# rrrickyz/Parallel-and-Distributed-Deep-Learning

Hardware: AMD Instinct MI355X
Metric: images/sec ResNet-50/ImageNet at 1/2/4/8 MI355X + scaling efficiency (higher is better)
Workload: dtype bf16; 1 GPU; model=ResNet-50 Keras-v1 (25,636,712 params, random init), global_batch=2560, per_gpu_batch=2560, image_size=224, parallelism=dp1, replicas=1, optimizer=adam, bn=frozen (training=False), hip_graph=False, grad_dtype=fp32, device=MI355X

## Files before the change

### csrc/bindings.cpp

```cpp
#include <torch/extension.h>

#include <atomic>
#include <ATen/hip/HIPContext.h>
#include <ATen/hip/impl/HIPGuardImplMasqueradingAsCUDA.h>
#include <c10/util/Optional.h>

#include "kernels/kernels.h"

using torch::Tensor;
using OptT = c10::optional<Tensor>;
namespace py = pybind11;

#define PCHECK(cond, msg) TORCH_CHECK(cond, "pddl: ", msg)

namespace {

std::atomic<bool> g_launched{false};
std::atomic<bool> g_knob_tuning{false};
hipStream_t cur_stream() {
  if (!g_launched.load(std::memory_order_relaxed)) g_launched.store(true, std::memory_order_relaxed);
  return at::hip::getCurrentHIPStream().stream();
}

void ok(const char* err, const char* what) { TORCH_CHECK(err == nullptr, "pddl ", what, ": ", err ? err : ""); }
// ... 802 lines not shown
  m.def("conv3x3c64_wgrad", &conv3x3c64_wgrad, REL, py::arg("x"), py::arg("g"), py::arg("dw"));
  m.def("c3c1", &c3c1, REL, py::arg("a"), py::arg("w3"), py::arg("scale3"), py::arg("shift3"),
        py::arg("res"), py::arg("out"), py::arg("bits3"), py::arg("w1"), py::arg("scale1"), py::arg("shift1"),
        py::arg("y1"), py::arg("bits1"));
  m.def("conv3x3c64_partial_rows", [](int64_t M) { return pddl::conv3x3c64_partial_rows((int)M); });
  m.def("gap_fwd", &gap_fwd, REL);
  m.def("gap_bwd", &gap_bwd, REL);
  m.def("colsum", &colsum, REL);
  m.def("softmax_xent", &softmax_xent, REL);
  m.def("eval_metrics", &eval_metrics, REL);
  m.def("colsum_reduce", &colsum_reduce, REL);
  m.def("allow_knob_changes", [](bool on) { g_knob_tuning.store(on); }, py::arg("on") = true);
  m.def("knobs_frozen", []() { return g_launched.load() && !g_knob_tuning.load(); });
  m.def("set_variant", [](const std::string& which, int v) {
    TORCH_CHECK(!g_launched.load() || g_knob_tuning.load(), "kernel knob ", which,
                ": knobs are read-only once a kernel has launched (set them before the first launch, "
                "e.g. PDDL_KNOBS, or call allow_knob_changes(True) in tuning code)");
    if (which == "igemm") pddl::g_igemm_variant = v;
    else if (which == "igemm_deep") pddl::g_igemm_deep = v;
    else if (which == "igemm_pf") pddl::g_igemm_pf = v;
    else if (which == "igemm8") pddl::g_igemm8 = v;
    else if (which == "igemm8_min_tiles") pddl::g_igemm8_min_tiles = v;
    else if (which == "wgrad8") pddl::g_wgrad8 = v;
    else if (which == "igemm_ns1_kt") pddl::g_igemm_ns1_kt = v;
    else if (which == "igemm8_min_n") pddl::g_igemm8_min_n = v;
    else if (which == "wgrad1") pddl::g_wgrad1 = v;
    else if (which == "igemm_n64") pddl::g_igemm_n64 = v;
    else if (which == "igemm_splitk") pddl::g_igemm_splitk = v;
    else if (which == "igemm_sk_fill") { TORCH_CHECK(v >= 1 && v <= 8, "igemm_sk_fill: 1-8"); pddl::g_igemm_sk_fill = v; }
    else if (which == "igemm_sk_cap") { TORCH_CHECK(v >= 2 && v <= 16, "igemm_sk_cap: 2-16"); pddl::g_igemm_sk_cap = v; }
    else if (which == "igemm_sk_elig") { TORCH_CHECK(v >= 1 && v <= 8, "igemm_sk_elig: 1-8"); pddl::g_igemm_sk_elig = v; }
    else if (which == "igemm_pk_all") pddl::g_igemm_pk_all = v;
    else if (which == "igemm_pk_dual") pddl::g_igemm_pk_dual = v;
    else if (which == "igemm_pk") { TORCH_CHECK(v == 0 || (v >= 2 && v <= 4), "igemm_pk: 0 or ring depth 2-4"); pddl::g_igemm_pk = v; }
    else if (which == "wgrad8_min_rows") { TORCH_CHECK(v >= 64, "wgrad8_min_rows"); pddl::g_wgrad8_min_rows = v; }
    else if (which == "stem") pddl::g_stem_variant = v;
    else if (which == "conv_f32") pddl::g_conv_f32_variant = v;
    else if (which == "conv_f32_splitk") pddl::g_conv_f32_splitk = v;
    else if (which == "conv_f32_sk_elig") { TORCH_CHECK(v >= 1 && v <= 8, "conv_f32_sk_elig: 1-8"); pddl::g_conv_f32_sk_elig = v; }
    else if (which == "wgrad_f32_wpc64") { TORCH_CHECK(v >= 1 && v <= 32, "wgrad_f32_wpc64"); pddl::g_wgrad_f32_wpc[0] = v; }
    else if (which == "wgrad_f32_wpc128") { TORCH_CHECK(v >= 1 && v <= 32, "wgrad_f32_wpc128"); pddl::g_wgrad_f32_wpc[1] = v; }
    else if (which == "c64_grid") pddl::g_c64_grid = v;
    else if (which == "c64w_grid") pddl::g_c64w_grid = v;
    else if (which == "bn_red_blocks") pddl::g_bn_red_blocks = v;
    else if (which == "bn_apply_blocks") pddl::g_bn_apply_blocks = v;
    else if (which == "pool_blocks") pddl::g_pool_blocks = v;
    else if (which == "colred_chunks") { TORCH_CHECK(v >= 1 && v <= 65535, "colred_chunks"); pddl::g_colred_chunks = v; }
    else TORCH_CHECK(false, "unknown kernel knob ", which);
  });
  m.def("wgrad_last_tiling", []() { return pddl::g_wgrad_last_tiling; });
  m.def("stream_capture_deps", [](int64_t stream) {
    hipStreamCaptureStatus st = hipStreamCaptureStatusNone;
    unsigned long long id = 0;
    hipGraph_t g = nullptr;
    const hipGraphNode_t* deps = nullptr;
    size_t n = 0;
    const hipError_t e = hipStreamGetCaptureInfo_v2(reinterpret_cast<hipStream_t>(stream), &st, &id, &g, &deps, &n);
    return std::make_tuple((int)e, (int)st, (int64_t)n);
  });
  m.def("igemm_partial_rows", [](int M, int Nn, int K, bool bnz) { return pddl::igemm_partial_rows(M, Nn, K, bnz); },
        py::arg("M"), py::arg("Nn"), py::arg("K"), py::arg("bnz") = false);
  m.def("igemm_splitk_floats", [](int M, int Nn, int K) { return (int64_t)pddl::igemm_splitk_floats(M, Nn, K); });
  m.def("splitk_use", &splitk_use, py::arg("workspace"));
  m.def("splitk_default_floats", &splitk_default_floats, py::arg("device"));
  m.def("igemm_plan", [](int M, int Nn, int K) {
    int cfg = 0, split = 0, ks = 1;
    pddl::igemm_plan_query(M, Nn, K, &cfg, &split, &ks);
    return std::make_tuple(cfg, split, ks);
  });
  m.def("maxpool_bwd_partial_rows", &pddl::maxpool_bwd_partial_rows);
  m.attr("COLRED_LAYER_BYTES") = (int)sizeof(pddl::ColRedLayer);
  m.def("prep", &prep, REL, py::arg("params"), py::arg("table"), py::arg("nlayers"), py::arg("max_elems"),
        py::arg("wbf"), py::arg("scale"), py::arg("shift"), py::arg("eps"), py::arg("parts") = 3);
  m.def("prep_fuse", &prep_fuse, REL);
  m.def("wgrad_finalize", &wgrad_finalize, REL, py::arg("params"), py::arg("grads"), py::arg("table"),
        py::arg("nlayers"), py::arg("scale"), py::arg("dgamma_raw"), py::arg("max_cout") = 2048);
  m.def("bn_grad", &bn_grad, REL);
  m.def("synth", &synth, REL);
  m.def("opt_hparams", &opt_hparams, REL);
  m.def("adam", &adam, REL);
  m.def("sgd", &sgd, REL);
  m.def("scale_", &scale_, REL);
  m.def("cast_bf16", &cast_bf16, REL);
// ... 10 lines not shown
```

### csrc/kernels/igemm.hip

```cpp
#include "common.h"
#include "kernels.h"

namespace pddl {

enum { AM_DIRECT = 0, AM_HALO = 1, AM_DUAL = 2 };

#ifndef IGEMM_MIN_BLOCKS
#define IGEMM_MIN_BLOCKS 2
#endif

__device__ __forceinline__ int sw_chunk(int lane, int i) { return (lane & 7) ^ ((4 * (i & 1) + (lane >> 4)) & 7); }
__device__ __forceinline__ int sw_read(int lane, int kh) { return (((kh * 4) + (lane >> 4)) ^ ((lane >> 1) & 7)) * 16; }

__device__ __forceinline__ uint32_t halo_taps(const IgemmParams& p, int hi, int wi) {
  if (p.R == 3 && p.S == 3) {
    const uint32_t cols = ((unsigned)wi < (unsigned)p.W ? 1u : 0u) | ((unsigned)(wi + 1) < (unsigned)p.W ? 2u : 0u) |
                          ((unsigned)(wi + 2) < (unsigned)p.W ? 4u : 0u);
    return ((unsigned)hi < (unsigned)p.H ? cols : 0u) | ((unsigned)(hi + 1) < (unsigned)p.H ? cols << 3 : 0u) |
           ((unsigned)(hi + 2) < (unsigned)p.H ? cols << 6 : 0u);
  }
  uint32_t rows = 0, cols = 0, mk = 0;
  for (int r = 0; r < p.R; ++r) rows |= (uint32_t)((unsigned)(hi + r) < (unsigned)p.H) << r;
  for (int s = 0; s < p.S; ++s) cols |= (uint32_t)((unsigned)(wi + s) < (unsigned)p.W) << s;
  for (int r = 0; r < p.R; ++r) mk |= ((rows >> r) & 1u) ? cols << (r * p.S) : 0u;
// ... 356 lines not shown
      for (int i = 0; i < TM; ++i)
#pragma unroll
        for (int j = 0; j < TN; ++j)
          acc[i][j] = __builtin_amdgcn_mfma_f32_16x16x32_bf16(af[i], bfr[j], acc[i][j], 0, 0, 0);
    }
    if (NSTAGE == 1 && t + 1 < KT) {
      __syncthreads();
      load_tile(0);
    }
    asm volatile("s_waitcnt vmcnt(0)" ::: "memory");
    __syncthreads();
  }

  if constexpr (SK) {
    float4* dst = reinterpret_cast<float4*>(p.slab) + ((long)(wg * ks + slice) * NW + wave) * (TM * TN) * 64 + lane;
#pragma unroll
    for (int i = 0; i < TM; ++i)
#pragma unroll
      for (int j = 0; j < TN; ++j)
        dst[(i * TN + j) * 64] = make_float4(acc[i][j][0], acc[i][j][1], acc[i][j][2], acc[i][j][3]);
    return;
  }

  float* stage = reinterpret_cast<float*>(smem) + wave * (32 * (WTN + 4));
  igemm_epilogue<TM, TN, PF, BNZ>(p, acc, m0 + wm * WTM, n0 + wn * WTN, p.prow_begin + tm * (BM / WTM) + wm, stage,
                                  lane);
}


typedef unsigned int v4u_t __attribute__((ext_vector_type(4)));
__device__ __forceinline__ int cdiv_signed(int a, int b) { return a >= 0 ? (a + b - 1) / b : -((-a) / b); }
__device__ __forceinline__ int pk_sw(int row) { return (row & 3) | ((row & 4) << 1); }

template <int KT, int NB, bool OPS, bool FWD, bool DUAL = false>
__global__ void __launch_bounds__(256, NB == 2 ? 2 : 1) igemm_pk_kernel(IgemmParams p) {
  constexpr int BM = 128, BN = 128, NW = 4, TM = 4, TN = 4, WAVES_N = 2;
  constexpr int A_BYTES = BM * 128, STAGE = A_BYTES + BN * 128;
  constexpr int BITS_BYTES = BM * 16;
  constexpr int AI = BM / (8 * NW), BI = BN / (8 * NW), PPS = AI + BI;
  constexpr int SPT = KT + (OPS ? 1 : 0);
  static_assert(NB >= 2 && NB * (STAGE + (OPS ? BITS_BYTES : 0)) <= 160 * 1024, "ring must fit the LDS");
  __shared__ __attribute__((aligned(16))) char smem[NB * STAGE + (OPS ? NB * BITS_BYTES : 1)];
  char* bits_lds = smem + NB * STAGE;
  const int tid = threadIdx.x, lane = tid & 63;
  const int wave = __builtin_amdgcn_readfirstlane(tid >> 6);
  const int wm = wave / WAVES_N, wn = wave % WAVES_N;
  const int mt = (p.M - p.m_begin + BM - 1) / BM, nt = (p.Nn + BN - 1) / BN;
  const int T = mt * nt, G = gridDim.x;
  const int bq = xcd_remap(blockIdx.x, G);
  if (bq >= T) return;
  const int t_begin = bq, t_end = T;
  const long HW = (long)p.H * p.W, pix_end = p.N * HW;
  const long HW2 = DUAL ? (long)p.H2 * p.W2 : 0;
  const int KT1 = DUAL ? p.K1 / 64 : KT;
  const int HoWo = p.Ho * p.Wo;
  const __amdgpu_buffer_rsrc_t rb = make_rsrc(p.b, p.Nn * p.ldb * 2);

  constexpr bool is_fwd = FWD;
  const uint16_t* opnd = is_fwd ? p.res : p.add;
  const int ld_op = is_fwd ? p.ld_res : p.ld_add;
  const bool res_on = OPS && opnd != nullptr;
  const bool bits_in = OPS && !is_fwd && p.bits_mask != nullptr;
  const bool bits_out = is_fwd && p.bits_out != nullptr;
  const bool csum_on = !is_fwd && p.colsum != nullptr;
  const int op_n = (res_on ? 8 : 0) + (bits_in ? 2 : 0) + (is_fwd ? 1 : 0);
  const int e_n = 2 * TM * (bits_out ? 2 : 1) + (csum_on ? 2 : 0);

  int ld_t = t_begin, ld_j = 0;
  uint32_t a_o[AI], a_o2[DUAL ? AI : 1], b_o[BI];
  __amdgpu_buffer_rsrc_t ra, ra2;
  auto set_tile = [&](int t) {
    const int m0 = p.m_begin + (t / nt) * BM, n0 = (t % nt) * BN;
    const int n_first = fdiv(m0, p.mg_howo);
    ra = make_rsrc_at(p.a1, n_first * HW * p.C1, pix_end * p.C1);
    if (DUAL) ra2 = make_rsrc_at(p.a2, n_first * HW2 * p.C2, p.N * HW2 * p.C2);
#pragma unroll
    for (int i = 0; i < AI; ++i) {
      const int m = m0 + (wave * AI + i) * 8 + (lane >> 3);
      a_o[i] = OOB_OFF;
      if (DUAL) a_o2[i] = OOB_OFF;
      if (m < p.M) {
        const int n = fdiv(m, p.mg_howo), rem = m - n * HoWo;
        const int ho = fdiv(rem, p.mg_wo), wo = rem - ho * p.Wo;
        const int pix = ((n - n_first) * p.H + ho * p.stride) * p.W + wo * p.stride;
        a_o[i] = (uint32_t)((pix * p.C1 + sw_chunk(lane, i) * 8) * 2);
        if (DUAL) {
          const int pix2 = ((n - n_first) * p.H2 + ho * p.stride2) * p.W2 + wo * p.stride2;
          a_o2[i] = (uint32_t)((pix2 * p.C2 + sw_chunk(lane, i) * 8) * 2);
        }
      }
    }
#pragma unroll
    for (int i = 0; i < BI; ++i) {
      const int n = n0 + (wave * BI + i) * 8 + (lane >> 3);
      b_o[i] = (n < p.Nn) ? (uint32_t)((n * p.ldb + sw_chunk(lane, i) * 8) * 2) : OOB_OFF;
    }
  };
  set_tile(t_begin);
  auto issue = [&](int buf) {
    const bool live = ld_t < t_end;
    char* base = smem + buf * STAGE;
    if (!OPS || ld_j < KT) {
      const int kofs = ld_j * 128;
      if (DUAL && ld_j >= KT1) {
#pragma unroll
        for (int i = 0; i < AI; ++i)
          buf_lds16(ra2, LDS_PTR(base + (wave * AI + i) * 1024), live ? a_o2[i] : OOB_OFF, kofs - KT1 * 128);
      } else {
#pragma unroll
        for (int i = 0; i < AI; ++i) buf_lds16(ra, LDS_PTR(base + (wave * AI + i) * 1024), live ? a_o[i] : OOB_OFF, kofs);
      }
#pragma unroll
      for (int i = 0; i < BI; ++i)
        buf_lds16(rb, LDS_PTR(base + A_BYTES + (wave * BI + i) * 1024), live ? b_o[i] : OOB_OFF, kofs);
    } else {
      const int lt = live ? ld_t : t_begin;
      const int m0 = p.m_begin + (lt / nt) * BM, n0 = (lt % nt) * BN;
      if (res_on) {
        const __amdgpu_buffer_rsrc_t ro = make_rsrc_at(opnd, (long)m0 * ld_op, (long)p.M * ld_op);
#pragma unroll
        for (int i = 0; i < 8; ++i) {
          const int row = wave * 32 + i * 4 + (lane >> 4);
          const int ch = (lane & 15) ^ pk_sw(row);
          const int col = n0 + ch * 8;
          const bool ok = live && m0 + row < p.M && col < p.Nn;
          buf_lds16(ro, LDS_PTR(base + (wave * 32 + i * 4) * 256), ok ? (uint32_t)((row * ld_op + col) * 2) : OOB_OFF, 0);
        }
      }
      if (is_fwd) {
        const float* src = wave < 2 ? p.scale : p.shift;
        const __amdgpu_buffer_rsrc_t rs = make_rsrc(src, p.Nn * 4);
        const int col = n0 + (wave & 1) * 64 + lane;
        __builtin_amdgcn_raw_ptr_buffer_load_lds(rs, LDS_PTR(bits_lds + buf * BITS_BYTES + wave * 256), 4,
                                                 live && col < p.Nn ? (uint32_t)(col * 4) : OOB_OFF, 0, 0, 0);
      }
      if (bits_in) {
        const int ldb8 = p.ld_bits_mask;
        const __amdgpu_buffer_rsrc_t rbm =
            __builtin_amdgcn_make_buffer_rsrc(const_cast<uint8_t*>(p.bits_mask) + (long)m0 * ldb8, (short)0,
                                              (int)lmin(((long)p.M - m0) * ldb8, 0x7fffffffL), 0x00020000);
#pragma unroll
        for (int q = 0; q < 2; ++q) {
          const int row = wave * 32 + q * 16 + (lane >> 2);
          const int byte = (n0 >> 3) + (lane & 3) * 4;
          const bool ok = live && m0 + row < p.M && byte * 8 < p.Nn;
          __builtin_amdgcn_raw_ptr_buffer_load_lds(rbm, LDS_PTR(bits_lds + buf * BITS_BYTES + (wave * 32 + q * 16) * 16), 4,
                                                   ok ? (uint32_t)(row * ldb8 + byte) : OOB_OFF, 0, 0, 0);
        }
      }
    }
    if (++ld_j == SPT) {
      ld_j = 0;
      ld_t += G;
      if (ld_t < t_end) set_tile(ld_t);
    }
  };
  auto wait_barrier = [&](int younger) {
    switch ((younger > 63 ? 63 : younger) >> 2) {
#define PK_W(n, c) case n: asm volatile("s_waitcnt vmcnt(" #c ") lgkmcnt(0)\n\ts_barrier" ::: "memory"); break;
      PK_W(1, 4) PK_W(2, 8) PK_W(3, 12) PK_W(4, 16) PK_W(5, 20) PK_W(6, 24) PK_W(7, 28) PK_W(8, 32) PK_W(9, 36)
      PK_W(10, 40) PK_W(11, 44) PK_W(12, 48) PK_W(13, 52) PK_W(14, 56) PK_W(15, 60)
#undef PK_W
      default: asm volatile("s_waitcnt vmcnt(0) lgkmcnt(0)\n\ts_barrier" ::: "memory"); break;
    }
  };

#pragma unroll
  for (int j = 0; j < NB - 1; ++j) issue(j);
  int cur = 0;
  const int a_off = (wm * 64 + (lane & 15)) * 128;
  const int b_off = (wn * 64 + (lane & 15)) * 128;
  const int g = lane >> 4, r = lane & 15, r8 = r & 7;
  const int lc = wn * 64 + 32 * (r >> 3) + 16 * (g & 1) + 8 * (g >> 1);
  for (int t = t_begin, u = 0; t < t_end; t += G, ++u) {
    const int m0 = p.m_begin + (t / nt) * BM, n0 = (t % nt) * BN;
    v4f acc[TM][TN];
#pragma unroll
    for (int i = 0; i < TM; ++i)
#pragma unroll
      for (int j = 0; j < TN; ++j) acc[i][j] = v4f{0.f, 0.f, 0.f, 0.f};
    int op_slot = 0;
#pragma unroll
    for (int j = 0; j < SPT; ++j) {
      int y = 0;
#pragma unroll
      for (int x = 1; x <= NB - 2; ++x) y += (OPS && (j + x) % SPT == KT) ? op_n : PPS;
      int ce = 1 - cdiv_signed(j - NB + 2, SPT);
      ce = ce < 0 ? 0 : (ce > u ? u : ce);
      wait_barrier(y + ce * e_n);
      issue(cur == 0 ? NB - 1 : cur - 1);
      if (!OPS || j < KT) {
        const char* As = smem + cur * STAGE;
        const char* Bs = As + A_BYTES;
#pragma unroll
        for (int kh = 0; kh < 2; ++kh) {
          const int pos = sw_read(lane, kh);
          v8bf af[TM], bfr[TN];
#pragma unroll
          for (int i = 0; i < TM; ++i) af[i] = *reinterpret_cast<const v8bf*>(As + a_off + i * 16 * 128 + pos);
#pragma unroll
          for (int jn = 0; jn < TN; ++jn) bfr[jn] = *reinterpret_cast<const v8bf*>(Bs + b_off + jn * 16 * 128 + pos);
#pragma unroll
          for (int i = 0; i < TM; ++i)
#pragma unroll
            for (int jn = 0; jn < TN; ++jn)
              acc[i][jn] = __builtin_amdgcn_mfma_f32_16x16x32_bf16(bfr[jn], af[i], acc[i][jn], 0, 0, 0);
        }
      } else {
        op_slot = cur;
      }
      cur = cur + 1 == NB ? 0 : cur + 1;
    }

#pragma unroll
    for (int i = 0; i < TM; ++i) {
#pragma unroll
      for (int q = 0; q < 2; ++q)
#pragma unroll
        for (int jj = 0; jj < 4; ++jj) {
          const auto sw = __builtin_amdgcn_permlane16_swap(__float_as_uint(acc[i][2 * q][jj]),
                                                           __float_as_uint(acc[i][2 * q + 1][jj]), false, false);
          acc[i][2 * q][jj] = __uint_as_float(sw[0]);
          acc[i][2 * q + 1][jj] = __uint_as_float(sw[1]);
        }
#pragma unroll
      for (int j = 0; j < 2; ++j)
#pragma unroll
        for (int jj = 0; jj < 4; ++jj) {
          const int c0 = __float_as_int(acc[i][j][jj]), c1 = __float_as_int(acc[i][2 + j][jj]);
          acc[i][j][jj] = __int_as_float(__builtin_amdgcn_update_dpp(c0, c1, 0x128, 0xf, 0xc, false));
          acc[i][2 + j][jj] = __int_as_float(__builtin_amdgcn_update_dpp(c1, c0, 0x128, 0xf, 0x3, false));
        }
    }
    const int gn = n0 + lc;
    const bool col_ok = gn < p.Nn;
    const char* bits_base = bits_lds + op_slot * BITS_BYTES;
    float sc[8], sh[8];
    if (is_fwd) {
      float4 a, b, c, d;
      const uint32_t sa = (uint32_t)(uintptr_t)LDS_PTR(bits_base + lc * 4);
      asm volatile("ds_read_b128 %0, %4\n\tds_read_b128 %1, %4 offset:16\n\t"
                   "ds_read_b128 %2, %4 offset:512\n\tds_read_b128 %3, %4 offset:528\n\ts_waitcnt lgkmcnt(0)"
                   : "=&v"(a), "=&v"(b), "=&v"(c), "=&v"(d) : "v"(sa) : "memory");
      sc[0] = a.x; sc[1] = a.y; sc[2] = a.z; sc[3] = a.w; sc[4] = b.x; sc[5] = b.y; sc[6] = b.z; sc[7] = b.w;
      sh[0] = c.x; sh[1] = c.y; sh[2] = c.z; sh[3] = c.w; sh[4] = d.x; sh[5] = d.y; sh[6] = d.z; sh[7] = d.w;
    }
    const __amdgpu_buffer_rsrc_t rout = make_rsrc_at(reinterpret_cast<const uint16_t*>(p.out), (long)m0 * p.ldo,
                                                     (long)p.M * p.ldo);
    const __amdgpu_buffer_rsrc_t rbo =
        __builtin_amdgcn_make_buffer_rsrc(bits_out ? p.bits_out + (long)m0 * p.ld_bits_out : reinterpret_cast<uint8_t*>(p.out),
                                          (short)0, bits_out ? (int)lmin(((long)p.M - m0) * p.ld_bits_out, 0x7fffffffL) : 0,
                                          0x00020000);
    char* op_w = smem + op_slot * STAGE;
    float csum[8] = {0.f, 0.f, 0.f, 0.f, 0.f, 0.f, 0.f, 0.f};
    uint32_t la[2 * TM];
#pragma unroll
    for (int k = 0; k < 2 * TM; ++k) {
      const int row = wm * 64 + 8 * k + r8;
      la[k] = (uint32_t)(uintptr_t)LDS_PTR(op_w + row * 256 + (((lc >> 3) ^ pk_sw(row)) << 4));
    }
    v4u_t ov4[2 * TM];
    uint32_t bytes[2 * TM];
    if (res_on) {
      asm volatile("ds_read_b128 %0, %8\n\tds_read_b128 %1, %9\n\tds_read_b128 %2, %10\n\tds_read_b128 %3, %11\n\t"
                   "ds_read_b128 %4, %12\n\tds_read_b128 %5, %13\n\tds_read_b128 %6, %14\n\tds_read_b128 %7, %15\n\t"
                   "s_waitcnt lgkmcnt(0)"
                   : "=&v"(ov4[0]), "=&v"(ov4[1]), "=&v"(ov4[2]), "=&v"(ov4[3]), "=&v"(ov4[4]), "=&v"(ov4[5]),
                     "=&v"(ov4[6]), "=&v"(ov4[7])
                   : "v"(la[0]), "v"(la[1]), "v"(la[2]), "v"(la[3]), "v"(la[4]), "v"(la[5]), "v"(la[6]), "v"(la[7])
                   : "memory");
    } else {
#pragma unroll
      for (int k = 0; k < 2 * TM; ++k) ov4[k] = v4u_t{0u, 0u, 0u, 0u};
    }
    if (bits_in) {
      uint32_t ba[2 * TM];
#pragma unroll
      for (int k = 0; k < 2 * TM; ++k)
        ba[k] = (uint32_t)(uintptr_t)LDS_PTR(bits_base + (wm * 64 + 8 * k + r8) * 16 + (lc >> 3));
      asm volatile("ds_read_u8 %0, %8\n\tds_read_u8 %1, %9\n\tds_read_u8 %2, %10\n\tds_read_u8 %3, %11\n\t"
                   "ds_read_u8 %4, %12\n\tds_read_u8 %5, %13\n\tds_read_u8 %6, %14\n\tds_read_u8 %7, %15\n\t"
                   "s_waitcnt lgkmcnt(0)"
                   : "=&v"(bytes[0]), "=&v"(bytes[1]), "=&v"(bytes[2]), "=&v"(bytes[3]), "=&v"(bytes[4]), "=&v"(bytes[5]),
                     "=&v"(bytes[6]), "=&v"(bytes[7])
                   : "v"(ba[0]), "v"(ba[1]), "v"(ba[2]), "v"(ba[3]), "v"(ba[4]), "v"(ba[5]), "v"(ba[6]), "v"(ba[7])
                   : "memory");
    }
#pragma unroll
    for (int i = 0; i < TM; ++i)
#pragma unroll
      for (int h = 0; h < 2; ++h) {
        const int k = 2 * i + h;
        float v[8];
#pragma unroll
        for (int e = 0; e < 4; ++e) { v[e] = acc[i][2 * h][e]; v[4 + e] = acc[i][2 * h + 1][e]; }
        float ov[8];
        unpack8(make_uint4(ov4[k].x, ov4[k].y, ov4[k].z, ov4[k].w), ov);
        uint4 pk;
        if constexpr (is_fwd) {
#pragma unroll
          for (int e = 0; e < 8; ++e) v[e] = v[e] * sc[e] + sh[e] + ov[e];
          pk = pack8(v);
          if (p.relu) pk = relu_pk8(pk);
        } else {
#pragma unroll
          for (int e = 0; e < 8; ++e) v[e] += ov[e];
          if (bits_in) {
#pragma unroll
            for (int e = 0; e < 8; ++e) v[e] = ((bytes[k] >> e) & 1u) ? v[e] : 0.f;
          }
          pk = pack8(v);
#pragma unroll
          for (int e = 0; e < 8; ++e) csum[e] += v[e];
        }
        const v4u_t pkv = {pk.x, pk.y, pk.z, pk.w};
        asm volatile("ds_write_b128 %0, %1" ::"v"(la[k]), "v"(pkv) : "memory");
      }
    uint32_t ra2[8];
#pragma unroll
    for (int it = 0; it < 8; ++it) {
      const int row = wm * 64 + it * 8 + (lane >> 3), c = wn * 8 + (lane & 7);
      ra2[it] = (uint32_t)(uintptr_t)LDS_PTR(op_w + row * 256 + ((c ^ pk_sw(row)) << 4));
    }
    v4u_t so[8];
    asm volatile("ds_read_b128 %0, %8\n\tds_read_b128 %1, %9\n\tds_read_b128 %2, %10\n\tds_read_b128 %3, %11\n\t"
                 "ds_read_b128 %4, %12\n\tds_read_b128 %5, %13\n\tds_read_b128 %6, %14\n\tds_read_b128 %7, %15\n\t"
                 "s_waitcnt lgkmcnt(0)"
                 : "=&v"(so[0]), "=&v"(so[1]), "=&v"(so[2]), "=&v"(so[3]), "=&v"(so[4]), "=&v"(so[5]), "=&v"(so[6]),
                   "=&v"(so[7])
                 : "v"(ra2[0]), "v"(ra2[1]), "v"(ra2[2]), "v"(ra2[3]), "v"(ra2[4]), "v"(ra2[5]), "v"(ra2[6]), "v"(ra2[7])
                 : "memory");
#pragma unroll
    for (int it = 0; it < 8; ++it) {
      const int row = wm * 64 + it * 8 + (lane >> 3), c = wn * 8 + (lane & 7);
      const int gc = n0 + c * 8;
      const bool ok = m0 + row < p.M && gc < p.Nn;
      __builtin_amdgcn_raw_buffer_store_b128(so[it], rout, ok ? (uint32_t)((row * p.ldo + gc) * 2) : OOB_OFF, 0, 0);
      if (bits_out)
        __builtin_amdgcn_raw_buffer_store_b8((unsigned char)pos_bits8(make_uint4(so[it].x, so[it].y, so[it].z, so[it].w)), rbo,
                                             ok ? (uint32_t)(row * p.ld_bits_out + (gc >> 3)) : OOB_OFF, 0, 0);
    }
    if (csum_on) {
#pragma unroll
      for (int o = 1; o < 8; o <<= 1)
#pragma unroll
        for (int e = 0; e < 8; ++e) csum[e] += __shfl_xor(csum[e], o, 64);
      const int prow = p.prow_begin + ((m0 - p.m_begin) / BM) * (BM / 64) + wm;
      const __amdgpu_buffer_rsrc_t rcs = __builtin_amdgcn_make_buffer_rsrc(p.colsum + (long)prow * p.Nn, (short)0,
                                                                           p.Nn * 4, 0x00020000);
      const bool w_ok = r8 == 0 && col_ok;
      typedef float v4fl __attribute__((ext_vector_type(4)));
      const v4fl c0 = {csum[0], csum[1], csum[2], csum[3]}, c1 = {csum[4], csum[5], csum[6], csum[7]};
      __builtin_amdgcn_raw_buffer_store_b128(__builtin_bit_cast(v4u_t, c0), rcs, w_ok ? (uint32_t)(gn * 4) : OOB_OFF, 0, 0);
      __builtin_amdgcn_raw_buffer_store_b128(__builtin_bit_cast(v4u_t, c1), rcs, w_ok ? (uint32_t)(gn * 4 + 16) : OOB_OFF,
                                             0, 0);
    }
  }
  asm volatile("s_waitcnt vmcnt(0)" ::: "memory");
}

template <int BM, int BN>
__global__ void __launch_bounds__(256) igemm_splitk_reduce_kernel(IgemmParams p) {
  constexpr int NW = 4, WTM = 64, WTN = 64, TM = 4, TN = 4, WAVES_N = BN / WTN, F = TM * TN;
  constexpr int EPI_LD = 16 + 4;
  __shared__ __attribute__((aligned(16))) float smem[4][32 * EPI_LD];
  const int lane = threadIdx.x & 63;
  const int jw = __builtin_amdgcn_readfirstlane(threadIdx.x >> 6);
// ... 253 lines not shown
  if (g_igemm_n64 == 1 && Nn % 128 && Nn % 64 == 0) return 0;
  if (g_igemm_n64 == 2 && K <= 64 && Nn % 64 == 0) return 0;
  if (g_igemm8 && Nn >= g_igemm8_min_n && K >= 256 && Nn < 4 * K && Nn % 256 == 0 &&
      (long)((M + 255) / 256) * ((Nn + 255) / 256) >= g_igemm8_min_tiles)
    return 4;
  return 1;
}
static int igemm_bm(int cfg) { return cfg == 1 ? 128 : 256; }

static int igemm_rows_of(int cfg, int m) {
  const int BM = igemm_bm(cfg);
  return ((m + BM - 1) / BM) * (BM / 64);
}

int num_cus() {
  static int cached[64] = {0};
  int dev = 0;
  if (hipGetDevice(&dev) != hipSuccess || dev < 0 || dev >= 64) return 256;
  if (!cached[dev]) {
    int n = 0;
    if (hipDeviceGetAttribute(&n, hipDeviceAttributeMultiprocessorCount, dev) != hipSuccess || n <= 0) n = 256;
    cached[dev] = n;
  }
  return cached[dev];
}

struct IgemmPlan { int cfg, split, ks; };

int g_igemm_splitk = 1;
int g_igemm_sk_fill = 2, g_igemm_sk_cap = 8, g_igemm_sk_elig = 2;
int g_igemm_pk = 2;
int g_igemm_pk_all = 0;

static int igemm_splitk_slices(int M, int Nn, int K, int cfg) {
  if (!g_igemm_splitk || (cfg != 0 && cfg != 1)) return 1;
  const int KT = K / 64;
  const int BM = igemm_bm(cfg), BN = cfg == 0 ? 64 : 128;
  const long T = (long)((M + BM - 1) / BM) * ((Nn + BN - 1) / BN);
  if (g_igemm_splitk >= 2) return KT >= 2 ? (g_igemm_splitk < KT ? g_igemm_splitk : KT) : 1;
  const long C = num_cus();
  const long target = (long)g_igemm_sk_fill * C;
  if (KT < 8) return 1;
  if ((long)g_igemm_sk_elig * T > C && !(T < target && KT >= 32)) return 1;
  long ks = (target + T - 1) / T;
  if (ks > KT / 4) ks = KT / 4;
  if (ks > g_igemm_sk_cap) ks = g_igemm_sk_cap;
  return ks >= 2 ? (int)ks : 1;
}

static IgemmPlan igemm_plan(int M, int Nn, int K, bool bnz = false) {
  IgemmPlan pl{igemm_config(M, Nn, K), M, 1};
  if (bnz) {
    if (pl.cfg != 0) pl.cfg = 1;
    return pl;
  }
  {
    const int c = pl.cfg == 4 ? 1 : pl.cfg;
    const int ks = igemm_splitk_slices(M, Nn, K, c);
    if (ks > 1) {
      pl.cfg = c;
      pl.ks = ks;
      return pl;
    }
  }
  if (pl.cfg != 4) return pl;
  const int nt = (Nn + 255) / 256, mt = (M + 255) / 256;
// ... 14 lines not shown
}

long igemm_splitk_floats(int M, int Nn, int K) {
  const IgemmPlan pl = igemm_plan(M, Nn, K);
  if (pl.ks <= 1) return 0;
  const int BM = igemm_bm(pl.cfg), BN = pl.cfg == 0 ? 64 : 128;
  return (long)((M + BM - 1) / BM) * ((Nn + BN - 1) / BN) * pl.ks * BM * BN;
}

int igemm_partial_rows(int M, int Nn, int K, bool bnz) {
  const IgemmPlan pl = igemm_plan(M, Nn, K, bnz);
  return igemm_rows_of(pl.cfg, pl.split) + (pl.split < M ? igemm_rows_of(1, M - pl.split) : 0);
}

static void igemm_launch_cfg(const IgemmParams& p, int cfg, hipStream_t stream);

int g_igemm_pk_dual = 2;
static bool igemm_pk_dual_launch(const IgemmParams& p, hipStream_t stream) {
  const int KT = p.K / 64;
  if (!g_igemm_pk_dual || KT > g_igemm_pk_dual || g_igemm_pk != 2) return false;
  if (p.mode != EPI_FWD || !p.scale || !p.shift || p.res || p.up2 || p.out2 || p.stats || p.bn_z) return false;
  if (p.R != 1 || p.S != 1 || p.pad != 0 || p.C1 != p.K1 || p.C2 != p.K - p.K1 || !igemm_no_halo(p)) return false;
  if (p.Nn % 32) return false;
  const long T = (long)((p.M - p.m_begin + 127) / 128) * ((p.Nn + 127) / 128);
  long G = (long)num_cus() * 2;
  if (G > T) G = T;
#define PKD_GO(KT_) hipLaunchKernelGGL((igemm_pk_kernel<KT_, 2, true, true, true>), dim3((unsigned)G), dim3(256), 0, stream, p)
  if (KT == 2) PKD_GO(2);
  else if (KT == 6) PKD_GO(6);
  else if (KT == 12) PKD_GO(12);
  else if (KT == 24) PKD_GO(24);
  else return false;
#undef PKD_GO
  return true;
}

static bool igemm_pk_launch(const IgemmParams& p, hipStream_t stream) {
  const int KT = p.K / 64;
  if (p.a2) return igemm_pk_dual_launch(p, stream);
  if (p.R != 1 || p.S != 1 || p.pad != 0 || p.C1 != p.K || !igemm_no_halo(p)) return false;
  if (KT != 1 && KT != 2 && KT != 4 && KT != 8) return false;
  if (p.mode != EPI_FWD && p.mode != EPI_DGRAD) return false;
  if (p.up2 || p.out2 || p.stats || p.bn_z || p.mask || p.Nn % 32) return false;
  if (p.mode == EPI_FWD && (!p.scale || !p.shift)) return false;
  const bool ops = p.mode == EPI_FWD || p.add || p.bits_mask;
  if (!ops) return false;
  if (!g_igemm_pk_all && !((p.mode == EPI_DGRAD && p.add) || (p.mode == EPI_FWD && p.res && KT >= 2))) return false;
  const long T = (long)((p.M - p.m_begin + 127) / 128) * ((p.Nn + 127) / 128);
  const int nb = g_igemm_pk;
  long G = (long)num_cus() * (nb == 2 ? 2 : 1);
  if (G > T) G = T;
#define PK_GO(KT_, NB_)                                                                                      \
  {                                                                                                          \
    if (p.mode == EPI_FWD) hipLaunchKernelGGL((igemm_pk_kernel<KT_, NB_, true, true>), dim3((unsigned)G), dim3(256), 0, stream, p); \
    else hipLaunchKernelGGL((igemm_pk_kernel<KT_, NB_, true, false>), dim3((unsigned)G), dim3(256), 0, stream, p); \
  }
#define PK_NB(KT_)                          \
  {                                         \
    if (nb == 2) PK_GO(KT_, 2)              \
    else if (nb == 3) PK_GO(KT_, 3)         \
    else PK_GO(KT_, 4)                      \
  }
  if (KT == 1) PK_NB(1) else if (KT == 2) PK_NB(2) else if (KT == 4) PK_NB(4) else PK_NB(8)
#undef PK_NB
#undef PK_GO
  return true;
}

const char* igemm_launch(const IgemmParams& p_in, hipStream_t stream) {
  const char* why = nullptr;
  if (!igemm_check(p_in, &why)) return why;
  IgemmParams p = p_in;
  p.mg_howo = fdiv_magic(p.Ho * p.Wo);
  p.mg_wo = fdiv_magic(p.Wo);
  p.m_begin = 0;
  p.prow_begin = 0;
  p.ksplit = 1;
  const IgemmPlan pl = igemm_plan(p.M, p.Nn, p.K, p.bn_z != nullptr);
  if (g_igemm_pk && pl.ks == 1 && ((pl.split >= p.M && pl.cfg == 1) || p.a2) && igemm_pk_launch(p, stream)) {
    hipError_t e = hipGetLastError();
    return e == hipSuccess ? nullptr : hipGetErrorString(e);
  }
  const bool window = (p.C1 * p.S == 64) && p.C1 < 64;
  if (pl.ks > 1 && !p.a2 && !window && p.C1 % 64 == 0 && p.slab && !(p.mode == EPI_FWD && p.up2) &&
      p.slab_floats >= igemm_splitk_floats(p.M, p.Nn, p.K)) {
    p.ksplit = pl.ks;
    const int BM = igemm_bm(pl.cfg), BN = pl.cfg == 0 ? 64 : 128;
    const int tiles = ((p.M + BM - 1) / BM) * ((p.Nn + BN - 1) / BN);
    igemm_launch_cfg(p, pl.cfg, stream);
    if (pl.cfg == 0) hipLaunchKernelGGL((igemm_splitk_reduce_kernel<256, 64>), dim3(tiles * 4), dim3(256), 0, stream, p);
    else hipLaunchKernelGGL((igemm_splitk_reduce_kernel<128, 128>), dim3(tiles * 4), dim3(256), 0, stream, p);
  } else if (pl.split < p.M) {
    IgemmParams head = p, tail = p;
    head.M = pl.split;
    tail.m_begin = pl.split;
    tail.prow_begin = igemm_rows_of(pl.cfg, pl.split);
    igemm_launch_cfg(head, pl.cfg, stream);
    igemm_launch_cfg(tail, 1, stream);
  } else {
    igemm_launch_cfg(p, pl.cfg, stream);
  }
  hipError_t e = hipGetLastError();
  return e == hipSuccess ? nullptr : hipGetErrorString(e);
}

static void igemm_launch_cfg(const IgemmParams& p, int cfg, hipStream_t stream) {
  const int KT = p.K / 64;
  int ns = g_igemm_variant;
  if (ns == 0) ns = KT <= g_igemm_ns1_kt ? 1 : 2;
  const int am = p.a2 ? AM_DUAL : (igemm_no_halo(p) ? AM_DIRECT : AM_HALO);
#define IG_GO(BM_, BN_, NS_, AM_) \
// ... 63 lines not shown
```

### csrc/kernels/kernels.h

```cpp
#pragma once
#include <hip/hip_runtime.h>
#include <stdint.h>

namespace pddl {

enum EpiMode { EPI_FWD = 0, EPI_DGRAD = 1, EPI_F32 = 2 };

struct IgemmParams {
  const uint16_t* a1; int C1;
  const uint16_t* a2; int C2;
  int H2, W2, stride2;
  int N, H, W;
  int R, S, stride, pad;
  int Ho, Wo, M;
  int K1, K;
  const uint16_t* b; int ldb; int Nn;
  int mode;
  const float* scale; const float* shift;
  const uint16_t* res; int ld_res;
  const uint16_t* mask; int ld_mask;
  const uint16_t* add; int ld_add;
  void* out; int ldo; int relu;
  void* out2; int ldo2; int relu2; int n_split;
  int up2; int Hf, Wf;
  float* colsum;
  uint8_t* bits_out; int ld_bits_out;
  const uint8_t* bits_mask; int ld_bits_mask;
  float* stats;
  const uint16_t* bn_z; const float* bn_mean;
  uint64_t mg_howo, mg_wo;
  int m_begin, prow_begin;
  float* slab; long slab_floats;
  int ksplit;
};
const char* igemm_launch(const IgemmParams& p, hipStream_t stream);
int igemm_partial_rows(int M, int Nn, int K, bool bnz = false);
void igemm_plan_query(int M, int Nn, int K, int* cfg, int* split, int* ksplit = nullptr);
long igemm_splitk_floats(int M, int Nn, int K);
extern int g_igemm8, g_igemm8_min_tiles, g_igemm8_min_n, g_igemm_ns1_kt, g_wgrad8, g_wgrad1;
int num_cus();
extern int g_wgrad_f32_wpc[2];
extern int g_wgrad_last_tiling;
extern int g_igemm_sk_fill, g_igemm_sk_cap, g_igemm_sk_elig;
extern int g_igemm_splitk, g_wgrad8_min_rows, g_igemm_pk, g_igemm_pk_all, g_igemm_pk_dual;
extern int g_stem_variant, g_igemm_n64, g_igemm_variant, g_igemm_deep, g_igemm_pf, g_bn_red_blocks, g_bn_apply_blocks, g_pool_blocks, g_colred_chunks;

struct WgradParams {
  const uint16_t* x; int N, H, W, C;
  int ldx;
  int R, S, stride, pad, Ho, Wo, M;
  const uint16_t* g; int ldg;
  const uint16_t* g2; int ldg2; int co_split;
  int Cout, K;
  float* dw; int ld_dw;
  int splits;
};
const char* wgrad_launch(const WgradParams& p, hipStream_t stream);

struct Bwd1x1Params {
  const uint16_t* g;
  const uint16_t* x;
  const uint16_t* wd; int ld_wd;
  const uint8_t* bits;
  uint16_t* out;
  float* colsum;
  float* dw; int ld_dw;
  int M, CO, CI;
  int s2, N, Hf, Wf, Hc, Wc;
  uint16_t* out2;
  uint64_t mg_hwc, mg_wc;
  const uint16_t* g1;
  const uint16_t* w1d;
  const uint8_t* gmask;
  uint16_t* gx;
  float* colsum_gx;
// ... 229 lines not shown
```

Before: 31450 images/sec.

## Add B-stationary variant of persistent ring igemm kernel keeping weights in registers

Adds a B-stationary variant of the persistent igemm_pk kernel for small-K (K=128/256) 1x1 convs. Each block loads its weight columns into VGPRs once, since the grid is a multiple of the N-tile count, and then streams only A tiles through the LDS ring, two K-chunks per stage. This is meant to remove repeated B loads into LDS and halve the pipeline steps per tile. In exchange it raises register pressure, and it splits the epilogue into smaller groups with scheduling barriers to compensate. It is enabled by default for forward K=256 shapes, and a debug query reports which kernel last ran.

```diff
diff --git a/csrc/bindings.cpp b/csrc/bindings.cpp
--- a/csrc/bindings.cpp
+++ b/csrc/bindings.cpp
@@ -858,6 +858,7 @@
     else if (which == "igemm_sk_elig") { TORCH_CHECK(v >= 1 && v <= 8, "igemm_sk_elig: 1-8"); pddl::g_igemm_sk_elig = v; }
     else if (which == "igemm_pk_all") pddl::g_igemm_pk_all = v;
     else if (which == "igemm_pk_dual") pddl::g_igemm_pk_dual = v;
+    else if (which == "igemm_pk_bstat") pddl::g_igemm_pk_bstat = v;
     else if (which == "igemm_pk") { TORCH_CHECK(v == 0 || (v >= 2 && v <= 4), "igemm_pk: 0 or ring depth 2-4"); pddl::g_igemm_pk = v; }
     else if (which == "wgrad8_min_rows") { TORCH_CHECK(v >= 64, "wgrad8_min_rows"); pddl::g_wgrad8_min_rows = v; }
     else if (which == "stem") pddl::g_stem_variant = v;
@@ -875,6 +876,9 @@
     else TORCH_CHECK(false, "unknown kernel knob ", which);
   });
   m.def("wgrad_last_tiling", []() { return pddl::g_wgrad_last_tiling; });
+  m.def("igemm_last_kernel", []() {
+    return std::string(pddl::g_igemm_last_kernel == 2 ? "ring_bstat" : pddl::g_igemm_last_kernel == 1 ? "ring" : "other");
+  });
   m.def("stream_capture_deps", [](int64_t stream) {
     hipStreamCaptureStatus st = hipStreamCaptureStatusNone;
     unsigned long long id = 0;
diff --git a/csrc/kernels/igemm.hip b/csrc/kernels/igemm.hip
--- a/csrc/kernels/igemm.hip
+++ b/csrc/kernels/igemm.hip
@@ -412,13 +412,16 @@
 __device__ __forceinline__ int cdiv_signed(int a, int b) { return a >= 0 ? (a + b - 1) / b : -((-a) / b); }
 __device__ __forceinline__ int pk_sw(int row) { return (row & 3) | ((row & 4) << 1); }
 
-template <int KT, int NB, bool OPS, bool FWD, bool DUAL = false>
+template <int KT, int NB, bool OPS, bool FWD, bool DUAL = false, bool BST = false>
 __global__ void __launch_bounds__(256, NB == 2 ? 2 : 1) igemm_pk_kernel(IgemmParams p) {
   constexpr int BM = 128, BN = 128, NW = 4, TM = 4, TN = 4, WAVES_N = 2;
   constexpr int A_BYTES = BM * 128, STAGE = A_BYTES + BN * 128;
   constexpr int BITS_BYTES = BM * 16;
   constexpr int AI = BM / (8 * NW), BI = BN / (8 * NW), PPS = AI + BI;
-  constexpr int SPT = KT + (OPS ? 1 : 0);
+  constexpr int KPS = BST ? 2 : 1;
+  constexpr int KS = KT / KPS;
+  constexpr int SPT = KS + (OPS ? 1 : 0);
+  static_assert(!BST || (!DUAL && KT % 2 == 0 && KT <= 4 && AI == BI), "B-stationary: single source, K = 128 / 256");
   static_assert(NB >= 2 && NB * (STAGE + (OPS ? BITS_BYTES : 0)) <= 160 * 1024, "ring must fit the LDS");
   __shared__ __attribute__((aligned(16))) char smem[NB * STAGE + (OPS ? NB * BITS_BYTES : 1)];
   char* bits_lds = smem + NB * STAGE;
@@ -447,11 +450,15 @@
   const int e_n = 2 * TM * (bits_out ? 2 : 1) + (csum_on ? 2 : 0);
 
   int ld_t = t_begin, ld_j = 0;
-  uint32_t a_o[AI], a_o2[DUAL ? AI : 1], b_o[BI];
+  uint32_t a_o[AI], a_o2[DUAL ? AI : 1], b_o[BST ? 1 : BI];
   __amdgpu_buffer_rsrc_t ra, ra2;
   auto set_tile = [&](int t) {
     const int m0 = p.m_begin + (t / nt) * BM, n0 = (t % nt) * BN;
-    const int n_first = fdiv(m0, p.mg_howo);
+    int lane = tid & 63;
+    uint64_t mg_howo = p.mg_howo, mg_wo = p.mg_wo;
+    int a_sn = p.H * p.W * p.C1 * 2, a_sh = p.stride * p.W * p.C1 * 2, a_sw = p.stride * p.C1 * 2;
+    if constexpr (BST) asm volatile("" : "+v"(lane), "+s"(mg_howo), "+s"(mg_wo), "+s"(a_sn), "+s"(a_sh), "+s"(a_sw));
+    const int n_first = fdiv(m0, mg_howo);
     ra = make_rsrc_at(p.a1, n_first * HW * p.C1, pix_end * p.C1);
     if (DUAL) ra2 = make_rsrc_at(p.a2, n_first * HW2 * p.C2, p.N * HW2 * p.C2);
 #pragma unroll
@@ -460,29 +467,55 @@
       a_o[i] = OOB_OFF;
       if (DUAL) a_o2[i] = OOB_OFF;
       if (m < p.M) {
-        const int n = fdiv(m, p.mg_howo), rem = m - n * HoWo;
-        const int ho = fdiv(rem, p.mg_wo), wo = rem - ho * p.Wo;
+        const int n = fdiv(m, mg_howo), rem = m - n * HoWo;
+        const int ho = fdiv(rem, mg_wo), wo = rem - ho * p.Wo;
         const int pix = ((n - n_first) * p.H + ho * p.stride) * p.W + wo * p.stride;
-        a_o[i] = (uint32_t)((pix * p.C1 + sw_chunk(lane, i) * 8) * 2);
+        if constexpr (BST) a_o[i] = (uint32_t)((n - n_first) * a_sn + ho * a_sh + wo * a_sw + sw_chunk(lane, i) * 16);
+        else a_o[i] = (uint32_t)((pix * p.C1 + sw_chunk(lane, i) * 8) * 2);
         if (DUAL) {
           const int pix2 = ((n - n_first) * p.H2 + ho * p.stride2) * p.W2 + wo * p.stride2;
           a_o2[i] = (uint32_t)((pix2 * p.C2 + sw_chunk(lane, i) * 8) * 2);
         }
       }
     }
-#pragma unroll
-    for (int i = 0; i < BI; ++i) {
-      const int n = n0 + (wave * BI + i) * 8 + (lane >> 3);
-      b_o[i] = (n < p.Nn) ? (uint32_t)((n * p.ldb + sw_chunk(lane, i) * 8) * 2) : OOB_OFF;
+    if constexpr (!BST) {
+#pragma unroll
+      for (int i = 0; i < BI; ++i) {
+        const int n = n0 + (wave * BI + i) * 8 + (lane >> 3);
+        b_o[i] = (n < p.Nn) ? (uint32_t)((n * p.ldb + sw_chunk(lane, i) * 8) * 2) : OOB_OFF;
+      }
     }
   };
+  v8bf bw[BST ? 2 * KT : 1][TN];
+  if constexpr (BST) {
+    const int nrow = (bq % nt) * BN + wn * 64 + (lane & 15);
+#pragma unroll
+    for (int ks = 0; ks < 2 * KT; ++ks)
+#pragma unroll
+      for (int jn = 0; jn < TN; ++jn) {
+        const int n = nrow + 16 * jn;
+        const uint32_t off = n < p.Nn ? (uint32_t)((n * p.ldb + 32 * ks + 8 * (lane >> 4)) * 2) : OOB_OFF;
+        bw[ks][jn] = __builtin_bit_cast(v8bf, __builtin_amdgcn_raw_buffer_load_b128(rb, off, 0, 0));
+      }
+    asm volatile("s_waitcnt vmcnt(0)" ::: "memory");
+#pragma unroll
+    for (int ks = 0; ks < 2 * KT; ++ks)
+#pragma unroll
+      for (int jn = 0; jn < TN; ++jn) asm volatile("" : "+v"(bw[ks][jn]));
+  }
   set_tile(t_begin);
   auto issue = [&](int buf) {
     const bool live = ld_t < t_end;
     char* base = smem + buf * STAGE;
-    if (!OPS || ld_j < KT) {
-      const int kofs = ld_j * 128;
-      if (DUAL && ld_j >= KT1) {
+    if (!OPS || ld_j < KS) {
+      const int kofs = ld_j * 128 * KPS;
+      if constexpr (BST) {
+#pragma unroll
+        for (int h = 0; h < 2; ++h)
+#pragma unroll
+          for (int i = 0; i < AI; ++i)
+            buf_lds16(ra, LDS_PTR(base + h * A_BYTES + (wave * AI + i) * 1024), live ? a_o[i] : OOB_OFF, kofs + h * 128);
+      } else if (DUAL && ld_j >= KT1) {
 #pragma unroll
         for (int i = 0; i < AI; ++i)
           buf_lds16(ra2, LDS_PTR(base + (wave * AI + i) * 1024), live ? a_o2[i] : OOB_OFF, kofs - KT1 * 128);
@@ -490,11 +523,15 @@
 #pragma unroll
         for (int i = 0; i < AI; ++i) buf_lds16(ra, LDS_PTR(base + (wave * AI + i) * 1024), live ? a_o[i] : OOB_OFF, kofs);
       }
-#pragma unroll
-      for (int i = 0; i < BI; ++i)
-        buf_lds16(rb, LDS_PTR(base + A_BYTES + (wave * BI + i) * 1024), live ? b_o[i] : OOB_OFF, kofs);
+      if constexpr (!BST) {
+#pragma unroll
+        for (int i = 0; i < BI; ++i)
+          buf_lds16(rb, LDS_PTR(base + A_BYTES + (wave * BI + i) * 1024), live ? b_o[i] : OOB_OFF, kofs);
+      }
     } else {
       const int lt = live ? ld_t : t_begin;
+      int lane = tid & 63;
+      if constexpr (BST) asm volatile("" : "+v"(lane));
       const int m0 = p.m_begin + (lt / nt) * BM, n0 = (lt % nt) * BN;
       if (res_on) {
         const __amdgpu_buffer_rsrc_t ro = make_rsrc_at(opnd, (long)m0 * ld_op, (long)p.M * ld_op);
@@ -550,10 +587,12 @@
   int cur = 0;
   const int a_off = (wm * 64 + (lane & 15)) * 128;
   const int b_off = (wn * 64 + (lane & 15)) * 128;
-  const int g = lane >> 4, r = lane & 15, r8 = r & 7;
-  const int lc = wn * 64 + 32 * (r >> 3) + 16 * (g & 1) + 8 * (g >> 1);
   for (int t = t_begin, u = 0; t < t_end; t += G, ++u) {
     const int m0 = p.m_begin + (t / nt) * BM, n0 = (t % nt) * BN;
+    int ln = lane;
+    if constexpr (BST) asm volatile("" : "+v"(ln));
+    const int g = ln >> 4, r = ln & 15, r8 = r & 7;
+    const int lc = wn * 64 + 32 * (r >> 3) + 16 * (g & 1) + 8 * (g >> 1);
     v4f acc[TM][TN];
 #pragma unroll
     for (int i = 0; i < TM; ++i)
@@ -564,27 +603,37 @@
     for (int j = 0; j < SPT; ++j) {
       int y = 0;
 #pragma unroll
-      for (int x = 1; x <= NB - 2; ++x) y += (OPS && (j + x) % SPT == KT) ? op_n : PPS;
+      for (int x = 1; x <= NB - 2; ++x) y += (OPS && (j + x) % SPT == KS) ? op_n : PPS;
       int ce = 1 - cdiv_signed(j - NB + 2, SPT);
       ce = ce < 0 ? 0 : (ce > u ? u : ce);
       wait_barrier(y + ce * e_n);
       issue(cur == 0 ? NB - 1 : cur - 1);
-      if (!OPS || j < KT) {
-        const char* As = smem + cur * STAGE;
-        const char* Bs = As + A_BYTES;
-#pragma unroll
-        for (int kh = 0; kh < 2; ++kh) {
-          const int pos = sw_read(lane, kh);
-          v8bf af[TM], bfr[TN];
-#pragma unroll
-          for (int i = 0; i < TM; ++i) af[i] = *reinterpret_cast<const v8bf*>(As + a_off + i * 16 * 128 + pos);
-#pragma unroll
-          for (int jn = 0; jn < TN; ++jn) bfr[jn] = *reinterpret_cast<const v8bf*>(Bs + b_off + jn * 16 * 128 + pos);
-#pragma unroll
-          for (int i = 0; i < TM; ++i)
-#pragma unroll
-            for (int jn = 0; jn < TN; ++jn)
-              acc[i][jn] = __builtin_amdgcn_mfma_f32_16x16x32_bf16(bfr[jn], af[i], acc[i][jn], 0, 0, 0);
+      if (!OPS || j < KS) {
+        int lk = lane;
+        if constexpr (BST) asm volatile("" : "+v"(lk));
+        const int a_off_k = BST ? (wm * 64 + (lk & 15)) * 128 : a_off;
+#pragma unroll
+        for (int h = 0; h < KPS; ++h) {
+          const char* As = smem + cur * STAGE + h * A_BYTES;
+          const char* Bs = smem + cur * STAGE + A_BYTES;
+#pragma unroll
+          for (int kh = 0; kh < 2; ++kh) {
+            const int pos = sw_read(lk, kh);
+            v8bf af[TM], bfr[TN];
+#pragma unroll
+            for (int i = 0; i < TM; ++i) af[i] = *reinterpret_cast<const v8bf*>(As + a_off_k + i * 16 * 128 + pos);
+#pragma unroll
+            for (int jn = 0; jn < TN; ++jn) {
+              if constexpr (BST) bfr[jn] = bw[(j * KPS + h) * 2 + kh][jn];
+              else bfr[jn] = *reinterpret_cast<const v8bf*>(Bs + b_off + jn * 16 * 128 + pos);
+            }
+#pragma unroll
+            for (int i = 0; i < TM; ++i)
+#pragma unroll
+              for (int jn = 0; jn < TN; ++jn)
+                acc[i][jn] = __builtin_amdgcn_mfma_f32_16x16x32_bf16(bfr[jn], af[i], acc[i][jn], 0, 0, 0);
+            if constexpr (BST && KT == 4) __builtin_amdgcn_sched_barrier(0);
+          }
         }
       } else {
         op_slot = cur;
@@ -633,49 +682,66 @@
                                           0x00020000);
     char* op_w = smem + op_slot * STAGE;
     float csum[8] = {0.f, 0.f, 0.f, 0.f, 0.f, 0.f, 0.f, 0.f};
-    uint32_t la[2 * TM];
-#pragma unroll
-    for (int k = 0; k < 2 * TM; ++k) {
-      const int row = wm * 64 + 8 * k + r8;
-      la[k] = (uint32_t)(uintptr_t)LDS_PTR(op_w + row * 256 + (((lc >> 3) ^ pk_sw(row)) << 4));
-    }
-    v4u_t ov4[2 * TM];
-    uint32_t bytes[2 * TM];
-    if (res_on) {
-      asm volatile("ds_read_b128 %0, %8\n\tds_read_b128 %1, %9\n\tds_read_b128 %2, %10\n\tds_read_b128 %3, %11\n\t"
-                   "ds_read_b128 %4, %12\n\tds_read_b128 %5, %13\n\tds_read_b128 %6, %14\n\tds_read_b128 %7, %15\n\t"
-                   "s_waitcnt lgkmcnt(0)"
-                   : "=&v"(ov4[0]), "=&v"(ov4[1]), "=&v"(ov4[2]), "=&v"(ov4[3]), "=&v"(ov4[4]), "=&v"(ov4[5]),
-                     "=&v"(ov4[6]), "=&v"(ov4[7])
-                   : "v"(la[0]), "v"(la[1]), "v"(la[2]), "v"(la[3]), "v"(la[4]), "v"(la[5]), "v"(la[6]), "v"(la[7])
-                   : "memory");
-    } else {
-#pragma unroll
-      for (int k = 0; k < 2 * TM; ++k) ov4[k] = v4u_t{0u, 0u, 0u, 0u};
-    }
-    if (bits_in) {
-      uint32_t ba[2 * TM];
-#pragma unroll
-      for (int k = 0; k < 2 * TM; ++k)
-        ba[k] = (uint32_t)(uintptr_t)LDS_PTR(bits_base + (wm * 64 + 8 * k + r8) * 16 + (lc >> 3));
-      asm volatile("ds_read_u8 %0, %8\n\tds_read_u8 %1, %9\n\tds_read_u8 %2, %10\n\tds_read_u8 %3, %11\n\t"
-                   "ds_read_u8 %4, %12\n\tds_read_u8 %5, %13\n\tds_read_u8 %6, %14\n\tds_read_u8 %7, %15\n\t"
-                   "s_waitcnt lgkmcnt(0)"
-                   : "=&v"(bytes[0]), "=&v"(bytes[1]), "=&v"(bytes[2]), "=&v"(bytes[3]), "=&v"(bytes[4]), "=&v"(bytes[5]),
-                     "=&v"(bytes[6]), "=&v"(bytes[7])
-                   : "v"(ba[0]), "v"(ba[1]), "v"(ba[2]), "v"(ba[3]), "v"(ba[4]), "v"(ba[5]), "v"(ba[6]), "v"(ba[7])
-                   : "memory");
-    }
-#pragma unroll
-    for (int i = 0; i < TM; ++i)
-#pragma unroll
-      for (int h = 0; h < 2; ++h) {
-        const int k = 2 * i + h;
+    constexpr int EG = BST && KT == 4 ? 2 : 2 * TM;
+#pragma unroll
+    for (int k0 = 0; k0 < 2 * TM; k0 += EG) {
+      uint32_t la[EG];
+#pragma unroll
+      for (int kk = 0; kk < EG; ++kk) {
+        const int row = wm * 64 + 8 * (k0 + kk) + r8;
+        la[kk] = (uint32_t)(uintptr_t)LDS_PTR(op_w + row * 256 + (((lc >> 3) ^ pk_sw(row)) << 4));
+      }
+      v4u_t ov4[EG];
+      uint32_t bytes[EG];
+      if (res_on) {
+        if constexpr (EG == 8) {
+          asm volatile("ds_read_b128 %0, %8\n\tds_read_b128 %1, %9\n\tds_read_b128 %2, %10\n\tds_read_b128 %3, %11\n\t"
+                       "ds_read_b128 %4, %12\n\tds_read_b128 %5, %13\n\tds_read_b128 %6, %14\n\tds_read_b128 %7, %15\n\t"
+                       "s_waitcnt lgkmcnt(0)"
+                       : "=&v"(ov4[0]), "=&v"(ov4[1]), "=&v"(ov4[2]), "=&v"(ov4[3]), "=&v"(ov4[4 % EG]), "=&v"(ov4[5 % EG]),
+                         "=&v"(ov4[6 % EG]), "=&v"(ov4[7 % EG])
+                       : "v"(la[0]), "v"(la[1]), "v"(la[2]), "v"(la[3]), "v"(la[4 % EG]), "v"(la[5 % EG]), "v"(la[6 % EG]),
+                         "v"(la[7 % EG])
+                       : "memory");
+        } else {
+          asm volatile("ds_read_b128 %0, %2\n\tds_read_b128 %1, %3\n\ts_waitcnt lgkmcnt(0)"
+                       : "=&v"(ov4[0]), "=&v"(ov4[1])
+                       : "v"(la[0]), "v"(la[1])
+                       : "memory");
+        }
+      } else {
+#pragma unroll
+        for (int kk = 0; kk < EG; ++kk) ov4[kk] = v4u_t{0u, 0u, 0u, 0u};
+      }
+      if (bits_in) {
+        uint32_t ba[EG];
+#pragma unroll
+        for (int kk = 0; kk < EG; ++kk)
+          ba[kk] = (uint32_t)(uintptr_t)LDS_PTR(bits_base + (wm * 64 + 8 * (k0 + kk) + r8) * 16 + (lc >> 3));
+        if constexpr (EG == 8) {
+          asm volatile("ds_read_u8 %0, %8\n\tds_read_u8 %1, %9\n\tds_read_u8 %2, %10\n\tds_read_u8 %3, %11\n\t"
+                       "ds_read_u8 %4, %12\n\tds_read_u8 %5, %13\n\tds_read_u8 %6, %14\n\tds_read_u8 %7, %15\n\t"
+                       "s_waitcnt lgkmcnt(0)"
+                       : "=&v"(bytes[0]), "=&v"(bytes[1]), "=&v"(bytes[2]), "=&v"(bytes[3]), "=&v"(bytes[4 % EG]),
+                         "=&v"(bytes[5 % EG]), "=&v"(bytes[6 % EG]), "=&v"(bytes[7 % EG])
+                       : "v"(ba[0]), "v"(ba[1]), "v"(ba[2]), "v"(ba[3]), "v"(ba[4 % EG]), "v"(ba[5 % EG]), "v"(ba[6 % EG]),
+                         "v"(ba[7 % EG])
+                       : "memory");
+        } else {
+          asm volatile("ds_read_u8 %0, %2\n\tds_read_u8 %1, %3\n\ts_waitcnt lgkmcnt(0)"
+                       : "=&v"(bytes[0]), "=&v"(bytes[1])
+                       : "v"(ba[0]), "v"(ba[1])
+                       : "memory");
+        }
+      }
+#pragma unroll
+      for (int kk = 0; kk < EG; ++kk) {
+        const int i = (k0 + kk) >> 1, h = (k0 + kk) & 1;
         float v[8];
 #pragma unroll
         for (int e = 0; e < 4; ++e) { v[e] = acc[i][2 * h][e]; v[4 + e] = acc[i][2 * h + 1][e]; }
         float ov[8];
-        unpack8(make_uint4(ov4[k].x, ov4[k].y, ov4[k].z, ov4[k].w), ov);
+        unpack8(make_uint4(ov4[kk].x, ov4[kk].y, ov4[kk].z, ov4[kk].w), ov);
         uint4 pk;
         if constexpr (is_fwd) {
 #pragma unroll
@@ -687,19 +753,21 @@
           for (int e = 0; e < 8; ++e) v[e] += ov[e];
           if (bits_in) {
 #pragma unroll
-            for (int e = 0; e < 8; ++e) v[e] = ((bytes[k] >> e) & 1u) ? v[e] : 0.f;
+            for (int e = 0; e < 8; ++e) v[e] = ((bytes[kk] >> e) & 1u) ? v[e] : 0.f;
           }
           pk = pack8(v);
 #pragma unroll
           for (int e = 0; e < 8; ++e) csum[e] += v[e];
         }
         const v4u_t pkv = {pk.x, pk.y, pk.z, pk.w};
-        asm volatile("ds_write_b128 %0, %1" ::"v"(la[k]), "v"(pkv) : "memory");
-      }
+        asm volatile("ds_write_b128 %0, %1" ::"v"(la[kk]), "v"(pkv) : "memory");
+      }
+      if constexpr (BST && KT == 4) __builtin_amdgcn_sched_barrier(0);
+    }
     uint32_t ra2[8];
 #pragma unroll
     for (int it = 0; it < 8; ++it) {
-      const int row = wm * 64 + it * 8 + (lane >> 3), c = wn * 8 + (lane & 7);
+      const int row = wm * 64 + it * 8 + (ln >> 3), c = wn * 8 + (ln & 7);
       ra2[it] = (uint32_t)(uintptr_t)LDS_PTR(op_w + row * 256 + ((c ^ pk_sw(row)) << 4));
     }
     v4u_t so[8];
@@ -712,7 +780,7 @@
                  : "memory");
 #pragma unroll
     for (int it = 0; it < 8; ++it) {
-      const int row = wm * 64 + it * 8 + (lane >> 3), c = wn * 8 + (lane & 7);
+      const int row = wm * 64 + it * 8 + (ln >> 3), c = wn * 8 + (ln & 7);
       const int gc = n0 + c * 8;
       const bool ok = m0 + row < p.M && gc < p.Nn;
       __builtin_amdgcn_raw_buffer_store_b128(so[it], rout, ok ? (uint32_t)((row * p.ldo + gc) * 2) : OOB_OFF, 0, 0);
@@ -1032,6 +1100,9 @@
 int g_igemm_pk = 2;
 int g_igemm_pk_all = 0;
 
+int g_igemm_pk_bstat = 1;
+int g_igemm_last_kernel = 0;
+
 static int igemm_splitk_slices(int M, int Nn, int K, int cfg) {
   if (!g_igemm_splitk || (cfg != 0 && cfg != 1)) return 1;
   const int KT = K / 64;
@@ -1112,6 +1183,7 @@
   else if (KT == 24) PKD_GO(24);
   else return false;
 #undef PKD_GO
+  g_igemm_last_kernel = 1;
   return true;
 }
 
@@ -1130,6 +1202,18 @@
   const int nb = g_igemm_pk;
   long G = (long)num_cus() * (nb == 2 ? 2 : 1);
   if (G > T) G = T;
+  const int nt = (p.Nn + 127) / 128;
+  const bool bst_shape = KT == 4 ? p.mode == EPI_FWD : (KT == 2 && g_igemm_pk_bstat >= 2);
+  if (g_igemm_pk_bstat && nb == 2 && bst_shape && G % nt == 0) {
+#define PK_BST(KT_, FWD_) \
+  hipLaunchKernelGGL((igemm_pk_kernel<KT_, 2, true, FWD_, false, true>), dim3((unsigned)G), dim3(256), 0, stream, p)
+    if (KT == 4) PK_BST(4, true);
+    else if (p.mode == EPI_FWD) PK_BST(2, true);
+    else PK_BST(2, false);
+#undef PK_BST
+    g_igemm_last_kernel = 2;
+    return true;
+  }
 #define PK_GO(KT_, NB_)                                                                                      \
   {                                                                                                          \
     if (p.mode == EPI_FWD) hipLaunchKernelGGL((igemm_pk_kernel<KT_, NB_, true, true>), dim3((unsigned)G), dim3(256), 0, stream, p); \
@@ -1144,6 +1228,7 @@
   if (KT == 1) PK_NB(1) else if (KT == 2) PK_NB(2) else if (KT == 4) PK_NB(4) else PK_NB(8)
 #undef PK_NB
 #undef PK_GO
+  g_igemm_last_kernel = 1;
   return true;
 }
 
@@ -1157,6 +1242,7 @@
   p.prow_begin = 0;
   p.ksplit = 1;
   const IgemmPlan pl = igemm_plan(p.M, p.Nn, p.K, p.bn_z != nullptr);
+  g_igemm_last_kernel = 0;
   if (g_igemm_pk && pl.ks == 1 && ((pl.split >= p.M && pl.cfg == 1) || p.a2) && igemm_pk_launch(p, stream)) {
     hipError_t e = hipGetLastError();
     return e == hipSuccess ? nullptr : hipGetErrorString(e);
diff --git a/csrc/kernels/kernels.h b/csrc/kernels/kernels.h
--- a/csrc/kernels/kernels.h
+++ b/csrc/kernels/kernels.h
@@ -41,6 +41,8 @@
 int num_cus();
 extern int g_wgrad_f32_wpc[2];
 extern int g_wgrad_last_tiling;
+extern int g_igemm_pk_bstat;
+extern int g_igemm_last_kernel;
 extern int g_igemm_sk_fill, g_igemm_sk_cap, g_igemm_sk_elig;
 extern int g_igemm_splitk, g_wgrad8_min_rows, g_igemm_pk, g_igemm_pk_all, g_igemm_pk_dual;
 extern int g_stem_variant, g_igemm_n64, g_igemm_variant, g_igemm_deep, g_igemm_pf, g_bn_red_blocks, g_bn_apply_blocks, g_pool_blocks, g_colred_chunks;
```

After: 31610 images/sec, median of 6. Within noise of the previous version (+0.5%).
